# fengpeng-yue/speech-to-speech-translation

Measured on AMD Instinct MI355X. Metric: mel-frames/sec (fwd+bwd+opt) on Fisher-shaped fbank80->mel80, higher is better.
Workload: dtype bf16; 1 GPU; s2st_transformer base 12enc/6dec d512 nfps4 + aux ASR/ST(1x64) + CTC, recipe dropouts, max-tokens=20000 Fisher-shaped batches, update-freq 1; parallelism=dp1

## Files before the change

include/s2st_hip.h:

```cpp
#ifndef S2ST_HIP_H
#define S2ST_HIP_H
#include <stdint.h>
#ifdef __cplusplus
extern "C" {
#endif

#define S2ST_OK 0
#define S2ST_ERR_LAUNCH (-1)
#define S2ST_ERR_SHAPE (-2)
#define S2ST_ERR_WORKSPACE (-3)
#define S2ST_ERR_ARG (-4)
#define S2ST_ERR_COMM (-5)

typedef struct { int64_t ld; int64_t bs; int32_t per; int32_t _pad; } s2st_split;

typedef struct {
  const void* p;
  int32_t kmajor;
  int32_t dtype;
  s2st_split sp;
  int64_t zo, zi;
} s2st_gemm_operand;

#define S2ST_F32 0
// ... 20 lines not shown
  float* colsum_part;
  int64_t bias_zo;
} s2st_gemm_epilogue;

typedef struct {
  s2st_gemm_operand A, B;
  s2st_gemm_out C;
  s2st_gemm_epilogue ep;
  int32_t M, N, K;
  int32_t batch, zdiv;
  int32_t precise;
  int32_t splitk, kchunk, avec, bvec, cvec, tiles_n;
  float* ws;
  int64_t ws_floats;
  float* slab;
} s2st_gemm_args;

int s2st_gemm_f32(const s2st_gemm_args* args, void* stream);
int s2st_gemm_tile_f32(const s2st_gemm_args* args, int32_t* tile, void* stream);

int64_t s2st_gemm_streamk_scratch_floats(void);
int s2st_gemm_streamk_scratch(float* scratch, int64_t floats, void* stream);

int s2st_gemm_group_f32(const s2st_gemm_args* list, int32_t n, void* stream);

typedef struct {
  int32_t error, form, bm, bn, splitk, kchunk, tiles_n, use_slab, vec, cvec, grid_x, grid_y, sk, n, total;
  int32_t cvec_of[8];
  char tag[104];
} s2st_gemm_plan_info;
int s2st_gemm_plan_f32(const s2st_gemm_args* args, int32_t ncu, int32_t slots160, int32_t sk_bound, s2st_gemm_plan_info* out);
int s2st_gemm_group_plan_f32(const s2st_gemm_args* list, int32_t n, int32_t ncu, int32_t slots160, int32_t sk_bound, s2st_gemm_plan_info* out);

typedef struct {
  const uint16_t *q, *k, *v;
  int64_t ldq, ldk, ldv;
  float* o;
// ... 408 lines not shown
```

speech-to-speech-translation_amd/csrc/c_api.cpp:

```cpp
#include <hip/hip_ext.h>
#include "s2st_ops.h"

extern "C" {

int s2st_version(void) { return 100; }

int s2st_experimental_build(void) {
#ifdef S2ST_EXPERIMENTAL
  return 1;
#else
  return 0;
#endif
}

int s2st_device_count(void) {
  int n = 0;
  if (hipGetDeviceCount(&n) != hipSuccess) return 0;
  return n;
}

int s2st_exchange_proxy_f32(const float* bucket, float* scratch, int64_t n, int64_t move_bytes, int32_t wgs, float gbps, void* stream) {
  return s2st_exchange_proxy(bucket, scratch, (long)n, (long)move_bytes, wgs, gbps, (hipStream_t)stream);
}
int s2st_grad_pack_bf16_f32(const float* g, uint16_t* out, int64_t n, void* stream) {
// ... 323 lines not shown
  return s2st_gemm_bf16_plan(a, 0, ncu, slots160, sk_bound != 0, out);
}
int s2st_gemm_group_plan_f32(const s2st_gemm_args* list, int32_t n, int32_t ncu, int32_t slots160, int32_t sk_bound, s2st_gemm_plan_info* out) {
  if (!list || n <= 0 || !out) return S2ST_ERR_ARG;
  return s2st_gemm_bf16_plan(list, n, ncu, slots160, sk_bound != 0, out);
}
int s2st_log_softmax_rows_f32(const float* x, int64_t ldx, float* y, int64_t ldy, int32_t rows, int32_t V, int32_t log_out, void* stream) {
  return s2st_log_softmax_rows(x, ldx, y, ldy, rows, V, log_out, (hipStream_t)stream);
}
int64_t s2st_gemm_streamk_scratch_floats(void) { return S2ST_STREAMK_SCRATCH_FLOATS; }
int s2st_gemm_streamk_scratch(float* scratch, int64_t floats, void* stream) {
  if (scratch && floats < S2ST_STREAMK_SCRATCH_FLOATS) return S2ST_ERR_WORKSPACE;
  s2st_gemm_streamk_bind((hipStream_t)stream, scratch, floats);
  return 0;
}
int s2st_w2v_wave_norm_f32(const float* x, const int32_t* lens, float* y, int32_t B, int32_t N, float eps, void* stream) {
  return s2st_w2v_wave_norm(x, lens, y, B, N, eps, (hipStream_t)stream);
}
int s2st_w2v_conv0_ln_gelu_f32(const float* wave, const float* w, const float* bias, const float* gamma, const float* beta, float* y, uint16_t* y_bf16, int32_t B, int32_t N, int32_t T, int32_t C, int32_t k, int32_t stride, float eps, void* stream) {
  return s2st_w2v_conv0_ln_gelu(wave, w, bias, gamma, beta, y, y_bf16, B, N, T, C, k, stride, eps, (hipStream_t)stream);
}
int s2st_w2v_ln_gelu_rows_f32(const float* x, const float* gamma, const float* beta, float* y, uint16_t* y_bf16, int32_t rows, int32_t C, float eps, void* stream) {
  return s2st_w2v_ln_gelu_rows(x, gamma, beta, y, y_bf16, rows, C, eps, (hipStream_t)stream);
}
int s2st_w2v_ctc_greedy_i32(const float* logits, const int32_t* lens, int32_t* ids, int32_t* counts, int32_t B, int32_t T, int32_t V, int32_t blank, void* stream) {
  return s2st_w2v_ctc_greedy(logits, lens, ids, counts, B, T, V, blank, (hipStream_t)stream);
}
int s2st_resample_sinc_f32(const float* x, const int32_t* n_in, const float* table, float* y, int32_t B, int32_t N_in, int32_t N_out, int32_t L, int32_t M, int32_t KL, int32_t KW, void* stream) {
  return s2st_resample_sinc(x, n_in, table, y, B, N_in, N_out, L, M, KL, KW, (hipStream_t)stream);
}
// ... 42 lines not shown
```

speech-to-speech-translation_amd/csrc/engine.cpp:

```cpp
#include <cmath>
#include <cstddef>
#include <cstdio>
#include <cstdlib>
#include <cstring>
#include <functional>
#include <string>
#include <vector>

#include "s2st_ops.h"
#include <hip/hip_ext.h>

namespace {

struct PInfo {
  std::string name;
  long off, numel;
  int ndim;
  int shape[4];
  int is_buffer;
};

struct Ten {
  float* d = nullptr;
  float* g = nullptr;
// ... 122 lines not shown
  float* dec_selfV(int l) const { return dec_selfK(l) + (long)dec_st.B * dec_st.maxT * c.dec_dim; }
  float* dec_crossKV(int l) const {
    return dec_st.base + (long)c.dec_layers * 2 * dec_st.B * dec_st.maxT * c.dec_dim + (long)l * dec_st.B * dec_st.E * 2 * c.dec_dim;
  }
  bool use_ln_skinny = true;
  bool use_skinny = true;
  bool use_ln_fuse = true;
  bool use_only_h = true;
  bool use_attn_gfuse = true;
  int attn_gfuse_mode = 1;
  bool ordered_sums = true;
  bool use_act_fuse = true;
  bool use_flash = true;
  bool attn_keep_f32 = s2st_env_on("S2ST_ATTN_KEEP_F32");
  bool convnet_fuse = s2st_env_int("S2ST_CONVNET_FUSE", 1) != 0;
  int ffn_act = 1;
  enum class Kind { Transformer, SpeechEncoder, HifiGan };
  Kind kind = Kind::Transformer;
  float* ws_for(hipStream_t s) const { return (side_ && s == side_) ? skws_side : skws; }
  float* skws = nullptr;
  long skws_n = 0;
  bool ph_fresh = false;
  bf16raw* PHT = nullptr;
  bool pht_valid = false;
  struct WT { long off; int N, K; };
  std::vector<WT> wt_list;
  void reg_wt(long off, int N, int K) { if (N % 8 == 0 && K % 8 == 0) wt_list.push_back(WT{off, N, K}); }
  bool has_wt(long off, int N, int K) const {
    if (!pht_valid) return false;
    for (const WT& t : wt_list) if (t.off == off && t.N == N && t.K == K) return true;
// ... 280 lines not shown
    if (rc == 0) {
      e->gscale = 1.f;
      for (int s = 0; s < e->n_segments(); ++s) e->backward_segment(s);
    }
    return rc;
  });
}

int s2st_engine_forward(s2st_engine* e, const s2st_batch* b, const s2st_outputs* out, float* workspace,
                        int64_t workspace_floats, void* stream) {
  if (!e->P || !e->BUF) return S2ST_ERR_ARG;
  e->begin_call(workspace, workspace_floats, stream);
  e->bt = *b;
  e->outs = *out;
  if (!e->outs.stats && b->tgt) return S2ST_ERR_ARG;
  return e->forward();
}

int s2st_engine_backward(s2st_engine* e, float gscale, int32_t segment, void* stream) {
  if (!e->G) return S2ST_ERR_ARG;
  e->st_ = (hipStream_t)stream;
  e->gscale = gscale;
  if (segment < 0) {
    for (int s = 0; s < e->n_segments(); ++s) {
      int rc = e->backward_segment(s);
      if (rc) return rc;
    }
    return 0;
  }
  return e->backward_segment(segment);
}

int s2st_engine_adam_overlapped(s2st_engine* e, float* exp_avg, float* exp_avg_sq, const float* sumsq_parts, int32_t n_parts,
                                float gmul, const float* gmul_dev, float max_norm, float lr, float beta1, float beta2, float eps,
                                float wd, int32_t step, float* gnorm_out, int32_t* skipped, int32_t write_bf16, int32_t n_chunks,
                                void* stream) {
  if (!e || !exp_avg || !exp_avg_sq || !sumsq_parts || n_parts <= 0) return S2ST_ERR_ARG;
// ... 305 lines not shown
```

speech-to-speech-translation_amd/csrc/gemm_bf16.hip:

```cpp
#include "gemm_bf16_tile.h"
#include "gemm_bf16_launch.h"

namespace {

template <int BM, int BN, bool AKM, bool BKM, bool VEC>
__global__ __launch_bounds__(256) void gemm_bf16_kernel(GemmArgs g) {
  constexpr int WM = BM / 2, WN = BN / 2, TM = WM / 16, TN = WN / 16;
  typedef Stage<AKM, BM, VEC> LA;
  typedef Stage<BKM, BN, VEC> LB;
  constexpr int A_BYTES = LA::BYTES, B_BYTES = LB::BYTES, STAGE = A_BYTES + B_BYTES;
  __shared__ __attribute__((aligned(16))) unsigned char smem[2 * STAGE];

  const int tid = threadIdx.x;
  const int wave = tid >> 6, lane = tid & 63;
  const int wm = wave >> 1, wn = wave & 1;

  const int nwg = gridDim.x;
  int id = blockIdx.x;
  {
    const int x = id & 7, q = nwg >> 3, r = nwg & 7;
    id = (x < r ? x * (q + 1) : r * (q + 1) + (x - r) * q) + (id >> 3);
  }
  const int tile_m = id / g.tiles_n, tile_n = id - tile_m * g.tiles_n;
  const int m0 = tile_m * BM, n0 = tile_n * BN;
// ... 190 lines not shown
#pragma unroll
        for (int i = 0; i < TM; ++i) {
#pragma unroll
          for (int j = 0; j < TN; ++j)
            acc[i][j] = __builtin_amdgcn_mfma_f32_16x16x32_bf16(bf[1][j], af[1][i], acc[i][j], 0, 0, 0);
#pragma unroll
          for (int q = (PER_STAGE * i) / TM; q < (PER_STAGE * (i + 1)) / TM; ++q) {
            if (q < DA::NI) da.issue_piece(nxt, kn, g.K, wave, q);
            else db.issue_piece(nxt + A_BYTES, kn, g.K, wave, q - DA::NI);
          }
          __builtin_amdgcn_sched_barrier(0);
        }
      }
    }
  }
  for (int t = t0; t < nt; ++t) {
    const int ahead = nt - 1 - t;
    if (ahead >= NS - 2) S2ST_VMCNT((NS - 2) * PER_STAGE);
    else if (NS > 3 && ahead == 1) S2ST_VMCNT(PER_STAGE);
    else S2ST_VMCNT(0);
    __builtin_amdgcn_s_barrier();
    unsigned char* cur = smem + (t % NS) * STAGE;
    if (t + NS - 1 < nt) {
      unsigned char* nxt = smem + ((t + NS - 1) % NS) * STAGE;
      da.issue(nxt, kbeg + (t + NS - 1) * BK, g.K, wave);
      db.issue(nxt + A_BYTES, kbeg + (t + NS - 1) * BK, g.K, wave);
    }
    if (t == nt - 1 && kend - (kbeg + t * BK) < BK) {
      const int kv = kend - (kbeg + t * BK);
      DA::sanitize(cur, kv, tid);
      DB::sanitize(cur + A_BYTES, kv, tid);
      __syncthreads();
    }
    bf16x8 af[2][TM], bf[2][TN];
    {
      typename LA::Raw ar[2][TM];
      typename LB::Raw br[2][TN];
#pragma unroll
      for (int s = 0; s < 2; ++s) {
#pragma unroll
        for (int j = 0; j < TN; ++j) br[s][j] = LB::raw(cur + A_BYTES, wn * WN + j * 16, s, lane);
#pragma unroll
// ... 4 lines not shown
      for (int s = 0; s < 2; ++s) {
#pragma unroll
        for (int j = 0; j < TN; ++j) bf[s][j] = LB::done(br[s][j]);
#pragma unroll
        for (int i = 0; i < TM; ++i) af[s][i] = LA::done(ar[s][i]);
      }
    }
    __builtin_amdgcn_sched_barrier(0);
#pragma unroll
    for (int s = 0; s < 2; ++s)
#pragma unroll
      for (int i = 0; i < TM; ++i)
#pragma unroll
        for (int j = 0; j < TN; ++j)
          acc[i][j] = __builtin_amdgcn_mfma_f32_16x16x32_bf16(bf[s][j], af[s][i], acc[i][j], 0, 0, 0);
  }
#ifdef S2ST_GEMM_STAMP
  stamp[3] = clock64();
#endif
  gemm_epilogue<BM, BN, WGN, IL>(g, acc, m0, n0, wm, wn, lane, zb, ks, zq, zr);
#ifdef S2ST_GEMM_STAMP
  stamp[4] = clock64();
  S2ST_VMCNT(0);
  stamp[5] = clock64();
  if (g.ws && tid == 0 && g.splitk == 1) {
    long* o = reinterpret_cast<long*>(g.ws) + (long)blockIdx.x * 8;
    for (int i = 0; i < 6; ++i) o[i] = stamp[i];
  }
#endif
}

template <int BM, int BN, bool AKM, bool BKM, int NS, int NW, bool IL = false>
__global__ __launch_bounds__(64 * NW) void gemm_bf16_dma_kernel(GemmArgs g) {
  gemm_bf16_dma_tile<BM, BN, AKM, BKM, NS, NW, IL>(g, (int)blockIdx.x, (int)gridDim.x, (int)blockIdx.y);
}
// ... 449 lines not shown
    sw.group_oneshot = s2st_env_int("S2ST_GROUP_ONESHOT", 1) != 0;
    return sw;
  }
  sw.p4 = s2st_env_int("S2ST_GEMM_P4", sw.p4);
  if (const char* force = s2st_env_str("S2ST_GEMM_TILE")) {
    sw.tile_set = true;
    if (sscanf(force, "%dx%d", &sw.tile_bm, &sw.tile_bn) != 2) sw.tile_bm = sw.tile_bn = 64;
  }
  return sw;
}

GemmChip gemm_chip(const GemmSwitches& sw, int ncu = 0, int slots160 = 0) {
  return GemmChip{ncu > 0 ? ncu : num_cus(sw), slots160 > 0 ? slots160 : s2st_gemm_bf16_w4_slots160(), kExperimental};
}

GemmGroup group_of(const GemmArgs* list, const GemmPlan& p) {
  GemmGroup grp{};
  grp.n = p.n;
  grp.total = p.total;
  for (int i = 0; i < p.n; ++i) {
    GemmArgs& g = grp.g[i] = list[i];
    if (g.zdiv <= 0) g.zdiv = 1;
    g.avec = g.bvec = p.vec;
    g.cvec = p.cvec_of[i];
    g.splitk = 1;
    g.slab = nullptr;
    g.kchunk = ((g.K + BK - 1) / BK) * BK;
    g.tiles_n = (g.N + p.bn - 1) / p.bn;
    grp.tile0[i + 1] = p.tile0[i + 1];
  }
  return grp;
}

}

void s2st_gemm_streamk_bind(hipStream_t st, float* scratch, long floats) {
  if (floats < S2ST_STREAMK_SCRATCH_FLOATS) scratch = nullptr;
  for (int i = 0; i < g_sk_n; ++i)
    if (g_sk[i].st == st) { g_sk[i].p = scratch; return; }
  if (g_sk_n < 4) g_sk[g_sk_n++] = SkScratch{st, scratch};
}
void s2st_gemm_streamk_unbind_all() { g_sk_n = 0; }

bool s2st_gemm_group_ok(const GemmArgs& g) {
  return group_member_ok(g, gemm_switches(SW_MEMBER));
}

int s2st_gemm_bf16_group(const GemmArgs* list, int n, hipStream_t st) {
  if (n <= 0) return 0;
  const GemmSwitches sw = gemm_switches(SW_GROUP);
  const GemmPlan p = plan_group(list, n, sw, gemm_chip(sw), sk_scratch(st) != nullptr);
  if (p.error) return p.error;
  GemmGroup grp = group_of(list, p);
  grp.xcd_global = 1;
  int rc = S2ST_ERR_ARG;
  switch (p.form) {
    case GEMM_GROUP_RING: rc = launch_group_ring(grp, st); break;
    case GEMM_GROUP_W4: rc = s2st_gemm_bf16_w4_group(grp, st); break;
#ifdef S2ST_EXPERIMENTAL
    case GEMM_GROUP_PERSISTENT: rc = launch_persistent<128, 128>(grp, p.sk, p.grid_x, st); break;
    case GEMM_GROUP_PERSISTENT_256: rc = launch_persistent<256, 128>(grp, p.sk, p.grid_x, st); break;
#endif
    default: break;
  }
  return rc == 0 && hipGetLastError() == hipSuccess ? 0 : S2ST_ERR_LAUNCH;
}

int s2st_gemm_bf16_preload(hipStream_t st) {
// ... 19 lines not shown
    rc |= launch_ring<256, 128>(g, grid, st);
#endif
    rc |= launch_group_ring(grp, st);
  }
  rc |= s2st_gemm_bf16_w4_preload(st);
  rc |= s2st_gemm_bf16_p4_preload(st);
  return rc || hipGetLastError() != hipSuccess ? -1 : 0;
}

int s2st_gemm_bf16(GemmArgs g, hipStream_t st, int* tile_out) {
  const GemmSwitches sw = gemm_switches(SW_SINGLE);
  const GemmPlan p = plan_single(g, sw, gemm_chip(sw), sk_scratch(st) != nullptr);
  if (p.error) return p.error;
  g.avec = g.bvec = p.vec;
  g.cvec = p.cvec;
  g.splitk = p.splitk;
  g.kchunk = p.kchunk;
  g.tiles_n = p.tiles_n;
  g.slab = p.use_slab ? g.ws : nullptr;
  if (tile_out) *tile_out = p.bm * 1000 + p.bn;
  const dim3 grid(p.grid_x, p.grid_y, 1);
  const bool wide = p.bn == 128;
  int rc = S2ST_ERR_ARG;
  switch (p.form) {
    case GEMM_STAGED:
      rc = !p.vec ? launch_staged<64, 64, false>(g, grid, st) : p.bm == 64 ? launch_staged<64, 64, true>(g, grid, st)
           : wide ? launch_staged<128, 128, true>(g, grid, st) : launch_staged<128, 64, true>(g, grid, st);
      break;
    case GEMM_RING:
      rc = p.bm == 160 ? launch_ring<160, 64>(g, grid, st) : p.bm == 64 ? launch_ring<64, 64>(g, grid, st)
           : wide ? launch_ring<128, 128>(g, grid, st) : launch_ring<128, 64>(g, grid, st);
      break;
    case GEMM_W4: rc = s2st_gemm_bf16_w4(g, p.bm, p.bn, grid, st); break;
    case GEMM_P4: rc = s2st_gemm_bf16_p4(g, grid, st); break;
#ifdef S2ST_EXPERIMENTAL
    case GEMM_RING_256x128: rc = launch_ring<256, 128>(g, grid, st); break;
    case GEMM_PERSISTENT:
      rc = wide ? launch_persistent<128, 128>(group_of(&g, p), p.sk, p.grid_x, st)
                : launch_persistent<128, 64>(group_of(&g, p), p.sk, p.grid_x, st);
      break;
#endif
    default: break;
  }
  if (rc) return rc;
  if (p.use_slab) {
    const long nthr = (long)g.M * ((g.N + 3) / 4);
    const double by = 4.0 * g.M * g.N * g.batch * (g.splitk + 1 + (g.ep.accumulate ? 1 : 0));
    s2st_launch("splitk_reduce_kernel", by, 0.0, splitk_reduce_kernel, dim3((unsigned)((nthr + 255) / 256), g.batch),
                dim3(256), 0, st, (const float*)g.slab, g.C, g.M, g.N, g.splitk, g.zdiv, g.ep.accumulate);
  }
  return hipGetLastError() == hipSuccess ? 0 : -1;
}

int s2st_gemm_bf16_plan(const GemmArgs* list, int n, int ncu, int slots160, bool sk_bound, s2st_gemm_plan_info* out) {
// ... 232 lines not shown
```

speech-to-speech-translation_amd/csrc/gemm_bf16_tile.h:

```cpp
#pragma once
#include <cstdio>
#include <cstdlib>

#include "s2st_ops.h"
#include "s2st_prof.h"

namespace {

typedef unsigned short bf16_t;
constexpr int BK = 64;

template <int ROWS>
__device__ __forceinline__ int kperm(int kr) {
  if (ROWS >= 128) return (kr & 3) | (((kr >> 3) & 1) << 2);
  return ((kr >> 1) & 1) | (((kr >> 3) & 1) << 1);
}

__device__ __forceinline__ uint4 mask_tail(uint4 v, int nvalid) {
  unsigned w[4] = {v.x, v.y, v.z, v.w};
#pragma unroll
  for (int i = 0; i < 4; ++i) {
    int e = nvalid - 2 * i;
    w[i] = e >= 2 ? w[i] : (e == 1 ? (w[i] & 0xffffu) : 0u);
  }
// ... 115 lines not shown
      const int kr = 32 * s + 8 * g + q;
      const unsigned char* a = img + kr * PITCH + ((((rt >> 4) ^ kperm<ROWS>(kr))) << 5) + 8 * p;
      s16x4 lo = lds_read_tr16(a);
      s16x4 hi = lds_read_tr16(a + 4 * PITCH);
      bf16x8 fr;
      fr[0] = lo[0]; fr[1] = lo[1]; fr[2] = lo[2]; fr[3] = lo[3];
      fr[4] = hi[0]; fr[5] = hi[1]; fr[6] = hi[2]; fr[7] = hi[3];
      return fr;
    }
  }
};

template <int BM, int BN, int WGN, bool DROP, bool RESID, bool ACC, bool HASC, bool HASH, bool H16, bool GELU = false>
__device__ __forceinline__ void gemm_epilogue_fast(const GemmArgs& g, f32x4 (&acc)[BM / 32][BN / (16 * WGN)], int m0, int n0,
                                                   int wm, int wn, int lane, int zb, int zq, int zr,
                                                   const float4 (*pre)[BN / (16 * WGN)]) {
  constexpr int WM = BM / 2, WN = BN / WGN, TM = WM / 16, TN = WN / 16;
  const long czoff = zq * g.C.zo + zr * g.C.zi;
  float* cbase = g.C.p + czoff;
  bf16_t* hbase = g.C.h + czoff;
  const float* rbase = g.ep.resid + czoff;
  const int M = g.M, N = g.N;
  const float alpha = g.ep.alpha, lo = g.ep.act == 1 ? 0.f : -__builtin_inff();
  const float drop_p = g.ep.drop_p, inv_keep = DROP ? 1.f / (1.f - drop_p) : 1.f;
  const uint64_t seed = g.ep.seed;
  int ncol[TN];
  bool nok[TN];
  float4 b4[TN];
#pragma unroll
  for (int j = 0; j < TN; ++j) {
    const int n = n0 + wn * WN + j * 16 + (lane >> 4) * 4;
    nok[j] = n < N;
    ncol[j] = nok[j] ? n : N - 4;
    b4[j] = make_float4(0.f, 0.f, 0.f, 0.f);
  }
  if (g.ep.bias) {
    const float* bias = g.ep.bias + zq * g.ep.bias_zo;
#pragma unroll
    for (int j = 0; j < TN; ++j) b4[j] = *reinterpret_cast<const float4*>(bias + ncol[j]);
  }
  long roff[TM];
  int mrow[TM];
  bool mok[TM];
#pragma unroll
  for (int i = 0; i < TM; ++i) {
    const int m = m0 + wm * WM + i * 16 + (lane & 15);
    mok[i] = m < M;
    mrow[i] = mok[i] ? m : M - 1;
    roff[i] = split_off(g.C.sp, mrow[i]);
  }
  float4 r4[RESID ? TM : 1][RESID ? TN : 1], c4[ACC ? TM : 1][ACC ? TN : 1];
  if (RESID) {
#pragma unroll
    for (int i = 0; i < TM; ++i)
#pragma unroll
      for (int j = 0; j < TN; ++j)
        r4[RESID ? i : 0][RESID ? j : 0] = pre ? pre[i][j] : *reinterpret_cast<const float4*>(rbase + roff[i] + ncol[j]);
  }
  if (ACC) {
#pragma unroll
    for (int i = 0; i < TM; ++i)
#pragma unroll
      for (int j = 0; j < TN; ++j)
        c4[ACC ? i : 0][ACC ? j : 0] = pre ? pre[i][j] : *reinterpret_cast<const float4*>(cbase + roff[i] + ncol[j]);
  }
  uint2 hp[(HASH && H16) ? TM : 1][(HASH && H16) ? TN : 1];
#pragma unroll
  for (int i = 0; i < TM; ++i) {
#pragma unroll
    for (int j = 0; j < TN; ++j) {
      float v[4] = {fmaxf(alpha * acc[i][j][0] + b4[j].x, lo), fmaxf(alpha * acc[i][j][1] + b4[j].y, lo),
                    fmaxf(alpha * acc[i][j][2] + b4[j].z, lo), fmaxf(alpha * acc[i][j][3] + b4[j].w, lo)};
      if (GELU) {
#pragma unroll
        for (int r = 0; r < 4; ++r) v[r] = gelu_erf_fast(v[r]);
      }
      if (DROP) {
        const uint64_t e0 = ((uint64_t)zb * M + mrow[i]) * (uint64_t)N + ncol[j];
#pragma unroll
// ... 27 lines not shown
        const bool ok = (odd ? mok[i + 1] : mok[i]) && n < N;
        const long ro = odd ? roff[i + 1] : roff[i];
        if (ok) *reinterpret_cast<uint4*>(hbase + ro + n) = make_uint4(ax, ay, bx, by);
      }
    }
    if constexpr (TM % 2 == 1) {
#pragma unroll
      for (int j = 0; j < TN; ++j)
        if (mok[TM - 1] && nok[j]) *reinterpret_cast<uint2*>(hbase + roff[TM - 1] + ncol[j]) = hp[TM - 1][j];
    }
  }
}

template <int BM, int BN, int WGN>
__device__ __forceinline__ void gemm_epilogue_fast_masky(const GemmArgs& g, f32x4 (&acc)[BM / 32][BN / (16 * WGN)], int m0, int n0,
                                                         int wm, int wn, int lane, int zq, int zr) {
  constexpr int WM = BM / 2, WN = BN / WGN, TM = WM / 16, TN = WN / 16;
  const long czoff = zq * g.C.zo + zr * g.C.zi;
  bf16_t* hbase = g.C.h + czoff;
  const bf16_t* ybase = g.ep.mask_y + czoff;
  const int M = g.M, N = g.N;
  const float alpha = g.ep.alpha * g.ep.mask_scale;
  int ncol[TN];
  bool nok[TN];
#pragma unroll
  for (int j = 0; j < TN; ++j) {
    const int n = n0 + wn * WN + j * 16 + (lane >> 4) * 4;
    nok[j] = n < N;
    ncol[j] = nok[j] ? n : N - 4;
  }
  long roff[TM];
  bool mok[TM];
  uint2 y4[TM][TN];
#pragma unroll
  for (int i = 0; i < TM; ++i) {
    const int m = m0 + wm * WM + i * 16 + (lane & 15);
    mok[i] = m < M;
    roff[i] = split_off(g.C.sp, mok[i] ? m : M - 1);
#pragma unroll
    for (int j = 0; j < TN; ++j) y4[i][j] = *reinterpret_cast<const uint2*>(ybase + roff[i] + ncol[j]);
  }
  float cs[TN][4];
#pragma unroll
  for (int j = 0; j < TN; ++j) cs[j][0] = cs[j][1] = cs[j][2] = cs[j][3] = 0.f;
  uint2 hp[TM][TN];
#pragma unroll
  for (int i = 0; i < TM; ++i) {
#pragma unroll
    for (int j = 0; j < TN; ++j) {
      const unsigned yw[4] = {y4[i][j].x & 0x7fffu, (y4[i][j].x >> 16) & 0x7fffu, y4[i][j].y & 0x7fffu, (y4[i][j].y >> 16) & 0x7fffu};
      float v[4];
#pragma unroll
      for (int r = 0; r < 4; ++r) {
        v[r] = yw[r] != 0 ? alpha * acc[i][j][r] : 0.f;
        if (mok[i] && nok[j]) cs[j][r] += v[r];
// ... 29 lines not shown
      for (int r = 0; r < 4; ++r) t[r] = row16_sum(cs[j][r]);
      if ((lane & 15) == 0 && nok[j]) {
        if (prow) *reinterpret_cast<float4*>(prow + ncol[j]) = make_float4(t[0], t[1], t[2], t[3]);
        else {
#pragma unroll
          for (int r = 0; r < 4; ++r) atomicAdd(g.ep.colsum + ncol[j] + r, t[r]);
        }
      }
    }
  }
}

template <int BM, int BN, int WGN, bool DROP, bool RESID, bool ACC, bool GELU = false>
__device__ __forceinline__ void gemm_epilogue_fast_out(const GemmArgs& g, f32x4 (&acc)[BM / 32][BN / (16 * WGN)], int m0, int n0,
                                                       int wm, int wn, int lane, int zb, int zq, int zr,
                                                       const float4 (*pre)[BN / (16 * WGN)]) {
  constexpr bool PAIRS = BM / 32 >= 2;
  if constexpr (ACC) {
    gemm_epilogue_fast<BM, BN, WGN, DROP, RESID, ACC, true, false, false>(g, acc, m0, n0, wm, wn, lane, zb, zq, zr, pre);
  } else {
    if (g.C.p && g.C.h) gemm_epilogue_fast<BM, BN, WGN, DROP, RESID, ACC, true, true, PAIRS, GELU>(g, acc, m0, n0, wm, wn, lane, zb, zq, zr, pre);
    else if (g.C.p) gemm_epilogue_fast<BM, BN, WGN, DROP, RESID, ACC, true, false, false, GELU>(g, acc, m0, n0, wm, wn, lane, zb, zq, zr, pre);
    else gemm_epilogue_fast<BM, BN, WGN, DROP, RESID, ACC, false, true, PAIRS, GELU>(g, acc, m0, n0, wm, wn, lane, zb, zq, zr, pre);
  }
}

template <int BM, int BN, int WGN, bool FAST = false>
__device__ __forceinline__ void gemm_epilogue(const GemmArgs& g, f32x4 (&acc)[BM / 32][BN / (16 * WGN)], int m0,
                                              int n0, int wm, int wn, int lane, int zb, int ks, int zq, int zr,
                                              const float4 (*pre)[BN / (16 * WGN)] = nullptr) {
  constexpr int WM = BM / 2, WN = BN / WGN, TM = WM / 16, TN = WN / 16;
  const long czoff = zq * g.C.zo + zr * g.C.zi;
  float* cbase = g.C.p ? g.C.p + czoff : nullptr;
  bf16_t* hbase = g.C.h ? g.C.h + czoff : nullptr;
  const float* rbase = g.ep.resid ? g.ep.resid + czoff : nullptr;
  const float inv_keep = g.ep.drop_p > 0.f ? 1.f / (1.f - g.ep.drop_p) : 1.f;
  const bool lead = (ks == 0);
  const bool cvec = g.cvec != 0;
  if constexpr (FAST) {
  if (g.cvec & 8) {
    gemm_epilogue_fast_masky<BM, BN, WGN>(g, acc, m0, n0, wm, wn, lane, zq, zr);
    return;
  }
  if (g.cvec & 2) {
    const bool drop = g.ep.drop_p > 0.f, res = g.ep.resid != nullptr, accu = g.ep.accumulate != 0;
    if (g.ep.act == 2) {
      if (res) gemm_epilogue_fast_out<BM, BN, WGN, false, true, false, true>(g, acc, m0, n0, wm, wn, lane, zb, zq, zr, pre);
      else gemm_epilogue_fast_out<BM, BN, WGN, false, false, false, true>(g, acc, m0, n0, wm, wn, lane, zb, zq, zr, pre);
    } else
    if (!drop && !res && !accu) gemm_epilogue_fast_out<BM, BN, WGN, false, false, false>(g, acc, m0, n0, wm, wn, lane, zb, zq, zr, pre);
    else if (!drop && res && !accu) gemm_epilogue_fast_out<BM, BN, WGN, false, true, false>(g, acc, m0, n0, wm, wn, lane, zb, zq, zr, pre);
    else if (!drop && !res && accu) gemm_epilogue_fast_out<BM, BN, WGN, false, false, true>(g, acc, m0, n0, wm, wn, lane, zb, zq, zr, pre);
    else if (drop && !res && !accu) gemm_epilogue_fast_out<BM, BN, WGN, true, false, false>(g, acc, m0, n0, wm, wn, lane, zb, zq, zr, pre);
    else gemm_epilogue_fast_out<BM, BN, WGN, true, true, false>(g, acc, m0, n0, wm, wn, lane, zb, zq, zr, pre);
    return;
  }
  }
  if (g.slab) {
    float* sb = g.slab + (long)blockIdx.y * g.M * g.N;
    const bool v4 = (g.N & 3) == 0;
#pragma unroll
    for (int i = 0; i < TM; ++i) {
      const int m = m0 + wm * WM + i * 16 + (lane & 15);
      if (m >= g.M) continue;
#pragma unroll
      for (int j = 0; j < TN; ++j) {
        const int n = n0 + wn * WN + j * 16 + (lane >> 4) * 4;
        if (n >= g.N) continue;
        float* dst = sb + (long)m * g.N + n;
// ... 204 lines not shown
```

speech-to-speech-translation_amd/csrc/s2st_ops.h:

```cpp
#pragma once
#include <cstdlib>
static inline const char* s2st_env_str(const char* name) { return getenv(name); }
static inline int s2st_env_int(const char* name, int dflt) { const char* e = getenv(name); return e ? atoi(e) : dflt; }
static inline bool s2st_env_on(const char* name) { return s2st_env_int(name, 0) != 0; }

#include <hip/hip_runtime.h>
#include <stdint.h>
#include "s2st_common.h"
#include "gemm_bf16_plan.h"

typedef s2st_gemm_out GemmOut;
typedef s2st_gemm_epilogue GemmEpilogue;

inline GemmOperand gemm_rowmajor(const float* p, long ld) {
  GemmOperand o;
  o.p = p; o.kmajor = 1; o.dtype = S2ST_F32; o.sp.ld = ld; o.sp.bs = 0; o.sp.per = 0; o.sp._pad = 0;
  o.zo = o.zi = 0;
  return o;
}
inline GemmOperand gemm_colmajor(const float* p, long ld) {
  GemmOperand o = gemm_rowmajor(p, ld);
  o.kmajor = 0;
  return o;
}
// ... 336 lines not shown
```

speech-to-speech-translation_amd/runtime/binding.py:

```python
from __future__ import annotations

import collections
import ctypes as C
import os
from typing import Optional

import torch

_HERE = os.path.dirname(os.path.abspath(__file__))
DEFAULT_LIB = os.path.join(os.path.dirname(_HERE), "csrc", "libs2st_hip.so")

_lib: Optional[C.CDLL] = None
_lib_is_emulator = False


class Split(C.Structure):
    _fields_ = [("ld", C.c_int64), ("bs", C.c_int64), ("per", C.c_int32), ("_pad", C.c_int32)]


class GemmOperand(C.Structure):
    _fields_ = [("p", C.c_void_p), ("kmajor", C.c_int32), ("dtype", C.c_int32), ("sp", Split),
                ("zo", C.c_int64), ("zi", C.c_int64)]


# ... 1 lines not shown
    _fields_ = [("p", C.c_void_p), ("sp", Split), ("zo", C.c_int64), ("zi", C.c_int64), ("h", C.c_void_p)]


class GemmEpilogue(C.Structure):
    _fields_ = [("alpha", C.c_float), ("act", C.c_int32), ("bias", C.c_void_p),
                ("drop_p", C.c_float), ("accumulate", C.c_int32), ("seed", C.c_uint64),
                ("resid", C.c_void_p), ("mask_y", C.c_void_p), ("mask_scale", C.c_float), ("colsum", C.c_void_p),
                ("colsum_part", C.c_void_p), ("bias_zo", C.c_int64)]


class GemmArgs(C.Structure):
    _fields_ = [("A", GemmOperand), ("B", GemmOperand), ("C", GemmOut), ("ep", GemmEpilogue),
                ("M", C.c_int32), ("N", C.c_int32), ("K", C.c_int32), ("batch", C.c_int32),
                ("zdiv", C.c_int32), ("precise", C.c_int32), ("splitk", C.c_int32),
                ("kchunk", C.c_int32), ("avec", C.c_int32), ("bvec", C.c_int32), ("cvec", C.c_int32),
                ("tiles_n", C.c_int32), ("ws", C.c_void_p), ("ws_floats", C.c_int64), ("slab", C.c_void_p)]


class S2STHipError(RuntimeError):
    pass


def load_library(path: Optional[str] = None, emulator: bool = False) -> C.CDLL:
    global _lib, _lib_is_emulator
    path = path or os.environ.get("S2ST_HIP_LIB") or DEFAULT_LIB
    if not os.path.exists(path):
        raise S2STHipError(
            f"{path} not found: build it with `python -c 'import __graft_entry__ as g; g.build()'`"
            " (hipcc --offload-arch=gfx950). There is no CPU fallback.")
    _lib = C.CDLL(path)
    _lib_is_emulator = emulator
# ... 309 lines not shown
```

Before: 1.511 million mel-frames/s.

## Prefetch GEMM epilogue operands early in the K-loop for training passes

During training forward and backward, a per-stream tail policy is bound so the bf16 GEMM kernel loads the epilogue operands (residual or accumulate source, bias, dropout mask) into registers at the start of the K loop. Those loads then overlap with the MFMA main loop instead of being fetched serially after it. The vmcnt waits are adjusted so the extra outstanding loads are not waited on each step. In exchange, more registers stay live through the main loop, which could reduce occupancy. It also adds global per-stream state and grows the args struct.

```diff
diff --git a/include/s2st_hip.h b/include/s2st_hip.h
--- a/include/s2st_hip.h
+++ b/include/s2st_hip.h
@@ -58,6 +58,8 @@
   float* ws;
   int64_t ws_floats;
   float* slab;
+  int32_t tail;
+  int32_t _pad_tail;
 } s2st_gemm_args;
 
 int s2st_gemm_f32(const s2st_gemm_args* args, void* stream);
@@ -65,6 +67,8 @@
 
 int64_t s2st_gemm_streamk_scratch_floats(void);
 int s2st_gemm_streamk_scratch(float* scratch, int64_t floats, void* stream);
+
+int s2st_stream_tail_policy(void* stream, int32_t mask);
 
 int s2st_gemm_group_f32(const s2st_gemm_args* list, int32_t n, void* stream);
 
diff --git a/speech-to-speech-translation_amd/csrc/c_api.cpp b/speech-to-speech-translation_amd/csrc/c_api.cpp
--- a/speech-to-speech-translation_amd/csrc/c_api.cpp
+++ b/speech-to-speech-translation_amd/csrc/c_api.cpp
@@ -361,6 +361,11 @@
   s2st_gemm_streamk_bind((hipStream_t)stream, scratch, floats);
   return 0;
 }
+int s2st_stream_tail_policy(void* stream, int32_t mask) {
+  if (mask < 0 || mask > S2ST_TAIL_EPI_EARLY) return S2ST_ERR_ARG;
+  s2st_tail_policy_bind((hipStream_t)stream, mask);
+  return 0;
+}
 int s2st_w2v_wave_norm_f32(const float* x, const int32_t* lens, float* y, int32_t B, int32_t N, float eps, void* stream) {
   return s2st_w2v_wave_norm(x, lens, y, B, N, eps, (hipStream_t)stream);
 }
diff --git a/speech-to-speech-translation_amd/csrc/engine.cpp b/speech-to-speech-translation_amd/csrc/engine.cpp
--- a/speech-to-speech-translation_amd/csrc/engine.cpp
+++ b/speech-to-speech-translation_amd/csrc/engine.cpp
@@ -160,6 +160,13 @@
   bool use_flash = true;
   bool attn_keep_f32 = s2st_env_on("S2ST_ATTN_KEEP_F32");
   bool convnet_fuse = s2st_env_int("S2ST_CONVNET_FUSE", 1) != 0;
+  struct TailScope {
+    hipStream_t st;
+    explicit TailScope(hipStream_t st_) : st(st_) {
+      s2st_tail_policy_bind(st, s2st_env_int("S2ST_EPI_EARLY", 1) != 0 ? S2ST_TAIL_EPI_EARLY : 0);
+    }
+    ~TailScope() { s2st_tail_policy_bind(st, 0); }
+  };
   int ffn_act = 1;
   enum class Kind { Transformer, SpeechEncoder, HifiGan };
   Kind kind = Kind::Transformer;
@@ -470,6 +477,8 @@
   e->bt = *b;
   e->outs = *out;
   if (!e->outs.stats && b->tgt) return S2ST_ERR_ARG;
+  if (!b->training) return e->forward();
+  s2st_engine::TailScope tail((hipStream_t)stream);
   return e->forward();
 }
 
@@ -477,6 +486,7 @@
   if (!e->G) return S2ST_ERR_ARG;
   e->st_ = (hipStream_t)stream;
   e->gscale = gscale;
+  s2st_engine::TailScope tail((hipStream_t)stream);
   if (segment < 0) {
     for (int s = 0; s < e->n_segments(); ++s) {
       int rc = e->backward_segment(s);
diff --git a/speech-to-speech-translation_amd/csrc/gemm_bf16.hip b/speech-to-speech-translation_amd/csrc/gemm_bf16.hip
--- a/speech-to-speech-translation_amd/csrc/gemm_bf16.hip
+++ b/speech-to-speech-translation_amd/csrc/gemm_bf16.hip
@@ -228,18 +228,8 @@
       }
     }
   }
-  for (int t = t0; t < nt; ++t) {
-    const int ahead = nt - 1 - t;
-    if (ahead >= NS - 2) S2ST_VMCNT((NS - 2) * PER_STAGE);
-    else if (NS > 3 && ahead == 1) S2ST_VMCNT(PER_STAGE);
-    else S2ST_VMCNT(0);
-    __builtin_amdgcn_s_barrier();
+  auto kstep = [&](int t) {
     unsigned char* cur = smem + (t % NS) * STAGE;
-    if (t + NS - 1 < nt) {
-      unsigned char* nxt = smem + ((t + NS - 1) % NS) * STAGE;
-      da.issue(nxt, kbeg + (t + NS - 1) * BK, g.K, wave);
-      db.issue(nxt + A_BYTES, kbeg + (t + NS - 1) * BK, g.K, wave);
-    }
     if (t == nt - 1 && kend - (kbeg + t * BK) < BK) {
       const int kv = kend - (kbeg + t * BK);
       DA::sanitize(cur, kv, tid);
@@ -274,11 +264,91 @@
 #pragma unroll
         for (int j = 0; j < TN; ++j)
           acc[i][j] = __builtin_amdgcn_mfma_f32_16x16x32_bf16(bf[s][j], af[s][i], acc[i][j], 0, 0, 0);
+  };
+  auto wait_stage = [&](int t) {
+    const int ahead = nt - 1 - t;
+    if (ahead >= NS - 2) S2ST_VMCNT((NS - 2) * PER_STAGE);
+    else if (NS > 3 && ahead == 1) S2ST_VMCNT(PER_STAGE);
+    else S2ST_VMCNT(0);
+  };
+  int t = t0;
+  float4 pre4[TM][TN], preb4[TN];
+  uint2 prey[TM][TN];
+  int early = 0;
+  if constexpr (IL) {
+    int ekind = 0;
+    if (g.tail & S2ST_TAIL_EPI_EARLY) {
+      if (g.cvec & 8) ekind = 3;
+      else if (g.cvec & 2) ekind = g.ep.accumulate ? 2 : g.ep.resid ? 1 : 0;
+    }
+    if (ekind != 0 && t < nt) {
+      wait_stage(t);
+      __builtin_amdgcn_s_barrier();
+      const long czoff = zq * g.C.zo + zr * g.C.zi;
+      int ncol[TN];
+      long roff[TM];
+#pragma unroll
+      for (int j = 0; j < TN; ++j) {
+        const int n = n0 + wn * WN + j * 16 + (lane >> 4) * 4;
+        ncol[j] = n < g.N ? n : g.N - 4;
+      }
+#pragma unroll
+      for (int i = 0; i < TM; ++i) {
+        const int m = m0 + wm * WM + i * 16 + (lane & 15);
+        roff[i] = split_off(g.C.sp, m < g.M ? m : g.M - 1) + czoff;
+      }
+      const bool ebias = ekind != 3 && g.ep.bias != nullptr;
+      __builtin_amdgcn_sched_barrier(0);
+      if (ekind == 3) {
+#pragma unroll
+        for (int i = 0; i < TM; ++i)
+#pragma unroll
+          for (int j = 0; j < TN; ++j) prey[i][j] = *reinterpret_cast<const uint2*>(g.ep.mask_y + roff[i] + ncol[j]);
+        early = 4;
+      } else {
+        const float* src = ekind == 2 ? g.C.p : g.ep.resid;
+#pragma unroll
+        for (int i = 0; i < TM; ++i)
+#pragma unroll
+          for (int j = 0; j < TN; ++j) pre4[i][j] = *reinterpret_cast<const float4*>(src + roff[i] + ncol[j]);
+        early = 1;
+        if (ebias) {
+          const float* bias = g.ep.bias + zq * g.ep.bias_zo;
+#pragma unroll
+          for (int j = 0; j < TN; ++j) preb4[j] = *reinterpret_cast<const float4*>(bias + ncol[j]);
+          early = 3;
+        }
+      }
+      __builtin_amdgcn_sched_barrier(0);
+      kstep(t);
+      for (++t; t < nt; ++t) {
+        const int ahead = nt - 1 - t;
+        if (ebias) {
+          if (NS > 3 && ahead == 1) S2ST_VMCNT(PER_STAGE + TM * TN + TN);
+          else S2ST_VMCNT(TM * TN + TN);
+        } else {
+          if (NS > 3 && ahead == 1) S2ST_VMCNT(PER_STAGE + TM * TN);
+          else S2ST_VMCNT(TM * TN);
+        }
+        __builtin_amdgcn_s_barrier();
+        kstep(t);
+      }
+    }
+  }
+  for (; t < nt; ++t) {
+    wait_stage(t);
+    __builtin_amdgcn_s_barrier();
+    if (t + NS - 1 < nt) {
+      unsigned char* nxt = smem + ((t + NS - 1) % NS) * STAGE;
+      da.issue(nxt, kbeg + (t + NS - 1) * BK, g.K, wave);
+      db.issue(nxt + A_BYTES, kbeg + (t + NS - 1) * BK, g.K, wave);
+    }
+    kstep(t);
   }
 #ifdef S2ST_GEMM_STAMP
   stamp[3] = clock64();
 #endif
-  gemm_epilogue<BM, BN, WGN, IL>(g, acc, m0, n0, wm, wn, lane, zb, ks, zq, zr);
+  gemm_epilogue<BM, BN, WGN, IL>(g, acc, m0, n0, wm, wn, lane, zb, ks, zq, zr, pre4, preb4, prey, early);
 #ifdef S2ST_GEMM_STAMP
   stamp[4] = clock64();
   S2ST_VMCNT(0);
@@ -758,7 +828,7 @@
   return GemmChip{ncu > 0 ? ncu : num_cus(sw), slots160 > 0 ? slots160 : s2st_gemm_bf16_w4_slots160(), kExperimental};
 }
 
-GemmGroup group_of(const GemmArgs* list, const GemmPlan& p) {
+GemmGroup group_of(const GemmArgs* list, const GemmPlan& p, hipStream_t st) {
   GemmGroup grp{};
   grp.n = p.n;
   grp.total = p.total;
@@ -767,6 +837,7 @@
     if (g.zdiv <= 0) g.zdiv = 1;
     g.avec = g.bvec = p.vec;
     g.cvec = p.cvec_of[i];
+    g.tail = s2st_tail_policy(st);
     g.splitk = 1;
     g.slab = nullptr;
     g.kchunk = ((g.K + BK - 1) / BK) * BK;
@@ -778,6 +849,24 @@
 
 }
 
+namespace {
+struct TailPolicy { hipStream_t st; int mask; };
+TailPolicy g_tail[8];
+int g_tail_n = 0;
+}
+int s2st_tail_policy(hipStream_t st) {
+  for (int i = 0; i < g_tail_n; ++i) if (g_tail[i].st == st) return g_tail[i].mask;
+  return 0;
+}
+void s2st_tail_policy_bind(hipStream_t st, int mask) {
+  for (int i = 0; i < g_tail_n; ++i)
+    if (g_tail[i].st == st) {
+      if (mask) g_tail[i].mask = mask;
+      else g_tail[i] = g_tail[--g_tail_n];
+      return;
+    }
+  if (mask && g_tail_n < 8) g_tail[g_tail_n++] = TailPolicy{st, mask};
+}
 void s2st_gemm_streamk_bind(hipStream_t st, float* scratch, long floats) {
   if (floats < S2ST_STREAMK_SCRATCH_FLOATS) scratch = nullptr;
   for (int i = 0; i < g_sk_n; ++i)
@@ -795,7 +884,7 @@
   const GemmSwitches sw = gemm_switches(SW_GROUP);
   const GemmPlan p = plan_group(list, n, sw, gemm_chip(sw), sk_scratch(st) != nullptr);
   if (p.error) return p.error;
-  GemmGroup grp = group_of(list, p);
+  GemmGroup grp = group_of(list, p, st);
   grp.xcd_global = 1;
   int rc = S2ST_ERR_ARG;
   switch (p.form) {
@@ -845,6 +934,7 @@
   if (p.error) return p.error;
   g.avec = g.bvec = p.vec;
   g.cvec = p.cvec;
+  g.tail = s2st_tail_policy(st);
   g.splitk = p.splitk;
   g.kchunk = p.kchunk;
   g.tiles_n = p.tiles_n;
@@ -867,8 +957,8 @@
 #ifdef S2ST_EXPERIMENTAL
     case GEMM_RING_256x128: rc = launch_ring<256, 128>(g, grid, st); break;
     case GEMM_PERSISTENT:
-      rc = wide ? launch_persistent<128, 128>(group_of(&g, p), p.sk, p.grid_x, st)
-                : launch_persistent<128, 64>(group_of(&g, p), p.sk, p.grid_x, st);
+      rc = wide ? launch_persistent<128, 128>(group_of(&g, p, st), p.sk, p.grid_x, st)
+                : launch_persistent<128, 64>(group_of(&g, p, st), p.sk, p.grid_x, st);
       break;
 #endif
     default: break;
diff --git a/speech-to-speech-translation_amd/csrc/gemm_bf16_tile.h b/speech-to-speech-translation_amd/csrc/gemm_bf16_tile.h
--- a/speech-to-speech-translation_amd/csrc/gemm_bf16_tile.h
+++ b/speech-to-speech-translation_amd/csrc/gemm_bf16_tile.h
@@ -153,7 +153,7 @@
 template <int BM, int BN, int WGN, bool DROP, bool RESID, bool ACC, bool HASC, bool HASH, bool H16, bool GELU = false>
 __device__ __forceinline__ void gemm_epilogue_fast(const GemmArgs& g, f32x4 (&acc)[BM / 32][BN / (16 * WGN)], int m0, int n0,
                                                    int wm, int wn, int lane, int zb, int zq, int zr,
-                                                   const float4 (*pre)[BN / (16 * WGN)]) {
+                                                   const float4 (*pre)[BN / (16 * WGN)], const float4* preb = nullptr, int early = 0) {
   constexpr int WM = BM / 2, WN = BN / WGN, TM = WM / 16, TN = WN / 16;
   const long czoff = zq * g.C.zo + zr * g.C.zi;
   float* cbase = g.C.p + czoff;
@@ -173,7 +173,10 @@
     ncol[j] = nok[j] ? n : N - 4;
     b4[j] = make_float4(0.f, 0.f, 0.f, 0.f);
   }
-  if (g.ep.bias) {
+  if (early & 2) {
+#pragma unroll
+    for (int j = 0; j < TN; ++j) b4[j] = preb[j];
+  } else if (g.ep.bias) {
     const float* bias = g.ep.bias + zq * g.ep.bias_zo;
 #pragma unroll
     for (int j = 0; j < TN; ++j) b4[j] = *reinterpret_cast<const float4*>(bias + ncol[j]);
@@ -190,18 +193,32 @@
   }
   float4 r4[RESID ? TM : 1][RESID ? TN : 1], c4[ACC ? TM : 1][ACC ? TN : 1];
   if (RESID) {
-#pragma unroll
-    for (int i = 0; i < TM; ++i)
-#pragma unroll
-      for (int j = 0; j < TN; ++j)
-        r4[RESID ? i : 0][RESID ? j : 0] = pre ? pre[i][j] : *reinterpret_cast<const float4*>(rbase + roff[i] + ncol[j]);
+    if (early & 1) {
+#pragma unroll
+      for (int i = 0; i < TM; ++i)
+#pragma unroll
+        for (int j = 0; j < TN; ++j) r4[RESID ? i : 0][RESID ? j : 0] = pre[i][j];
+    } else {
+#pragma unroll
+      for (int i = 0; i < TM; ++i)
+#pragma unroll
+        for (int j = 0; j < TN; ++j)
+          r4[RESID ? i : 0][RESID ? j : 0] = *reinterpret_cast<const float4*>(rbase + roff[i] + ncol[j]);
+    }
   }
   if (ACC) {
-#pragma unroll
-    for (int i = 0; i < TM; ++i)
-#pragma unroll
-      for (int j = 0; j < TN; ++j)
-        c4[ACC ? i : 0][ACC ? j : 0] = pre ? pre[i][j] : *reinterpret_cast<const float4*>(cbase + roff[i] + ncol[j]);
+    if (early & 1) {
+#pragma unroll
+      for (int i = 0; i < TM; ++i)
+#pragma unroll
+        for (int j = 0; j < TN; ++j) c4[ACC ? i : 0][ACC ? j : 0] = pre[i][j];
+    } else {
+#pragma unroll
+      for (int i = 0; i < TM; ++i)
+#pragma unroll
+        for (int j = 0; j < TN; ++j)
+          c4[ACC ? i : 0][ACC ? j : 0] = *reinterpret_cast<const float4*>(cbase + roff[i] + ncol[j]);
+    }
   }
   uint2 hp[(HASH && H16) ? TM : 1][(HASH && H16) ? TN : 1];
 #pragma unroll
@@ -259,7 +276,8 @@
 
 template <int BM, int BN, int WGN>
 __device__ __forceinline__ void gemm_epilogue_fast_masky(const GemmArgs& g, f32x4 (&acc)[BM / 32][BN / (16 * WGN)], int m0, int n0,
-                                                         int wm, int wn, int lane, int zq, int zr) {
+                                                         int wm, int wn, int lane, int zq, int zr,
+                                                         const uint2 (*prey)[BN / (16 * WGN)] = nullptr, int early = 0) {
   constexpr int WM = BM / 2, WN = BN / WGN, TM = WM / 16, TN = WN / 16;
   const long czoff = zq * g.C.zo + zr * g.C.zi;
   bf16_t* hbase = g.C.h + czoff;
@@ -282,8 +300,17 @@
     const int m = m0 + wm * WM + i * 16 + (lane & 15);
     mok[i] = m < M;
     roff[i] = split_off(g.C.sp, mok[i] ? m : M - 1);
-#pragma unroll
-    for (int j = 0; j < TN; ++j) y4[i][j] = *reinterpret_cast<const uint2*>(ybase + roff[i] + ncol[j]);
+  }
+  if (early & 4) {
+#pragma unroll
+    for (int i = 0; i < TM; ++i)
+#pragma unroll
+      for (int j = 0; j < TN; ++j) y4[i][j] = prey[i][j];
+  } else {
+#pragma unroll
+    for (int i = 0; i < TM; ++i)
+#pragma unroll
+      for (int j = 0; j < TN; ++j) y4[i][j] = *reinterpret_cast<const uint2*>(ybase + roff[i] + ncol[j]);
   }
   float cs[TN][4];
 #pragma unroll
@@ -343,21 +370,22 @@
 template <int BM, int BN, int WGN, bool DROP, bool RESID, bool ACC, bool GELU = false>
 __device__ __forceinline__ void gemm_epilogue_fast_out(const GemmArgs& g, f32x4 (&acc)[BM / 32][BN / (16 * WGN)], int m0, int n0,
                                                        int wm, int wn, int lane, int zb, int zq, int zr,
-                                                       const float4 (*pre)[BN / (16 * WGN)]) {
+                                                       const float4 (*pre)[BN / (16 * WGN)], const float4* preb, int early) {
   constexpr bool PAIRS = BM / 32 >= 2;
   if constexpr (ACC) {
-    gemm_epilogue_fast<BM, BN, WGN, DROP, RESID, ACC, true, false, false>(g, acc, m0, n0, wm, wn, lane, zb, zq, zr, pre);
+    gemm_epilogue_fast<BM, BN, WGN, DROP, RESID, ACC, true, false, false>(g, acc, m0, n0, wm, wn, lane, zb, zq, zr, pre, preb, early);
   } else {
-    if (g.C.p && g.C.h) gemm_epilogue_fast<BM, BN, WGN, DROP, RESID, ACC, true, true, PAIRS, GELU>(g, acc, m0, n0, wm, wn, lane, zb, zq, zr, pre);
-    else if (g.C.p) gemm_epilogue_fast<BM, BN, WGN, DROP, RESID, ACC, true, false, false, GELU>(g, acc, m0, n0, wm, wn, lane, zb, zq, zr, pre);
-    else gemm_epilogue_fast<BM, BN, WGN, DROP, RESID, ACC, false, true, PAIRS, GELU>(g, acc, m0, n0, wm, wn, lane, zb, zq, zr, pre);
+    if (g.C.p && g.C.h) gemm_epilogue_fast<BM, BN, WGN, DROP, RESID, ACC, true, true, PAIRS, GELU>(g, acc, m0, n0, wm, wn, lane, zb, zq, zr, pre, preb, early);
+    else if (g.C.p) gemm_epilogue_fast<BM, BN, WGN, DROP, RESID, ACC, true, false, false, GELU>(g, acc, m0, n0, wm, wn, lane, zb, zq, zr, pre, preb, early);
+    else gemm_epilogue_fast<BM, BN, WGN, DROP, RESID, ACC, false, true, PAIRS, GELU>(g, acc, m0, n0, wm, wn, lane, zb, zq, zr, pre, preb, early);
   }
 }
 
 template <int BM, int BN, int WGN, bool FAST = false>
 __device__ __forceinline__ void gemm_epilogue(const GemmArgs& g, f32x4 (&acc)[BM / 32][BN / (16 * WGN)], int m0,
                                               int n0, int wm, int wn, int lane, int zb, int ks, int zq, int zr,
-                                              const float4 (*pre)[BN / (16 * WGN)] = nullptr) {
+                                              const float4 (*pre)[BN / (16 * WGN)] = nullptr, const float4* preb = nullptr,
+                                              const uint2 (*prey)[BN / (16 * WGN)] = nullptr, int early = 0) {
   constexpr int WM = BM / 2, WN = BN / WGN, TM = WM / 16, TN = WN / 16;
   const long czoff = zq * g.C.zo + zr * g.C.zi;
   float* cbase = g.C.p ? g.C.p + czoff : nullptr;
@@ -368,20 +396,20 @@
   const bool cvec = g.cvec != 0;
   if constexpr (FAST) {
   if (g.cvec & 8) {
-    gemm_epilogue_fast_masky<BM, BN, WGN>(g, acc, m0, n0, wm, wn, lane, zq, zr);
+    gemm_epilogue_fast_masky<BM, BN, WGN>(g, acc, m0, n0, wm, wn, lane, zq, zr, prey, early);
     return;
   }
   if (g.cvec & 2) {
     const bool drop = g.ep.drop_p > 0.f, res = g.ep.resid != nullptr, accu = g.ep.accumulate != 0;
     if (g.ep.act == 2) {
-      if (res) gemm_epilogue_fast_out<BM, BN, WGN, false, true, false, true>(g, acc, m0, n0, wm, wn, lane, zb, zq, zr, pre);
-      else gemm_epilogue_fast_out<BM, BN, WGN, false, false, false, true>(g, acc, m0, n0, wm, wn, lane, zb, zq, zr, pre);
+      if (res) gemm_epilogue_fast_out<BM, BN, WGN, false, true, false, true>(g, acc, m0, n0, wm, wn, lane, zb, zq, zr, pre, preb, early);
+      else gemm_epilogue_fast_out<BM, BN, WGN, false, false, false, true>(g, acc, m0, n0, wm, wn, lane, zb, zq, zr, pre, preb, early);
     } else
-    if (!drop && !res && !accu) gemm_epilogue_fast_out<BM, BN, WGN, false, false, false>(g, acc, m0, n0, wm, wn, lane, zb, zq, zr, pre);
-    else if (!drop && res && !accu) gemm_epilogue_fast_out<BM, BN, WGN, false, true, false>(g, acc, m0, n0, wm, wn, lane, zb, zq, zr, pre);
-    else if (!drop && !res && accu) gemm_epilogue_fast_out<BM, BN, WGN, false, false, true>(g, acc, m0, n0, wm, wn, lane, zb, zq, zr, pre);
-    else if (drop && !res && !accu) gemm_epilogue_fast_out<BM, BN, WGN, true, false, false>(g, acc, m0, n0, wm, wn, lane, zb, zq, zr, pre);
-    else gemm_epilogue_fast_out<BM, BN, WGN, true, true, false>(g, acc, m0, n0, wm, wn, lane, zb, zq, zr, pre);
+    if (!drop && !res && !accu) gemm_epilogue_fast_out<BM, BN, WGN, false, false, false>(g, acc, m0, n0, wm, wn, lane, zb, zq, zr, pre, preb, early);
+    else if (!drop && res && !accu) gemm_epilogue_fast_out<BM, BN, WGN, false, true, false>(g, acc, m0, n0, wm, wn, lane, zb, zq, zr, pre, preb, early);
+    else if (!drop && !res && accu) gemm_epilogue_fast_out<BM, BN, WGN, false, false, true>(g, acc, m0, n0, wm, wn, lane, zb, zq, zr, pre, preb, early);
+    else if (drop && !res && !accu) gemm_epilogue_fast_out<BM, BN, WGN, true, false, false>(g, acc, m0, n0, wm, wn, lane, zb, zq, zr, pre, preb, early);
+    else gemm_epilogue_fast_out<BM, BN, WGN, true, true, false>(g, acc, m0, n0, wm, wn, lane, zb, zq, zr, pre, preb, early);
     return;
   }
   }
diff --git a/speech-to-speech-translation_amd/csrc/s2st_ops.h b/speech-to-speech-translation_amd/csrc/s2st_ops.h
--- a/speech-to-speech-translation_amd/csrc/s2st_ops.h
+++ b/speech-to-speech-translation_amd/csrc/s2st_ops.h
@@ -7,6 +7,9 @@
 #include <hip/hip_runtime.h>
 #include <stdint.h>
 #include "s2st_common.h"
+#define S2ST_TAIL_EPI_EARLY 1
+int s2st_tail_policy(hipStream_t st);
+void s2st_tail_policy_bind(hipStream_t st, int mask);
 #include "gemm_bf16_plan.h"
 
 typedef s2st_gemm_out GemmOut;
diff --git a/speech-to-speech-translation_amd/runtime/binding.py b/speech-to-speech-translation_amd/runtime/binding.py
--- a/speech-to-speech-translation_amd/runtime/binding.py
+++ b/speech-to-speech-translation_amd/runtime/binding.py
@@ -39,7 +39,8 @@
                 ("M", C.c_int32), ("N", C.c_int32), ("K", C.c_int32), ("batch", C.c_int32),
                 ("zdiv", C.c_int32), ("precise", C.c_int32), ("splitk", C.c_int32),
                 ("kchunk", C.c_int32), ("avec", C.c_int32), ("bvec", C.c_int32), ("cvec", C.c_int32),
-                ("tiles_n", C.c_int32), ("ws", C.c_void_p), ("ws_floats", C.c_int64), ("slab", C.c_void_p)]
+                ("tiles_n", C.c_int32), ("ws", C.c_void_p), ("ws_floats", C.c_int64), ("slab", C.c_void_p),
+                ("tail", C.c_int32), ("_pad_tail", C.c_int32)]
 
 
 class S2STHipError(RuntimeError):
```

New measurement: 1.461 million mel-frames/s. -3.3%, worse.
